# spotify/basic-pitch

Measured on NVIDIA H100. Metric: audio_seconds_per_second, higher is better.
Workload: dtype f32

## Files before the change

### basic_pitch_b200/_lib.py

```python
from __future__ import annotations

import ctypes as C
import os
import pathlib
from typing import Optional

LIB_PATH = pathlib.Path(__file__).resolve().parent / "libbp_b200.so"

BP_OK = 0
BP_E_INVALID = -1
BP_E_CUDA = -2
BP_E_CAPACITY = -3
BP_E_NOMEM = -4

EXPORTS = [
    "bp_version", "bp_last_error", "bp_default_decode_params", "bp_num_windows", "bp_num_frames",
    "bp_model_create", "bp_model_destroy", "bp_model_device", "bp_model_param_block", "bp_model_refresh",
    "bp_model_launch_count", "bp_forward_device", "bp_forward_host", "bp_run_inference_device",
    "bp_run_inference_host", "bp_decode_device", "bp_decode_host", "bp_transcribe_host", "bp_transcribe_device",
    "bp_infer_onsets_host", "bp_pitch_bends_host", "bp_debug_activation", "bp_model_chunk_windows", "bp_model_set_path", "bp_model_profile", "bp_model_profile_read", "bp_debug_tc_plan", "bp_debug_tc_gather", "bp_debug_tc_gather_packed", "bp_debug_tc_b2", "bp_debug_tc_clocks", "bp_transcribe_files_host", "bp_host_alloc", "bp_host_free", "bp_last_required", "bp_resampled_length", "bp_load_pcm_device", "bp_load_pcm_host", "bp_debug_resample_filter", "bp_write_note_files", "bp_sonify_notes_host", "bp_load_pcm_files_device", "bp_transcribe_pcm_files_host", "bp_debug_pcm_layout", "bp_debug_frontend", "bp_model_set_debug_frontend", "bp_debug_chain_layout", "bp_debug_split_layout", "bp_decode_grid_device", "bp_decode_grid_host", "bp_decode_grid_chunk_params", "bp_default_score_params", "bp_frame_times", "bp_score_grid_device", "bp_score_grid_host", "bp_score_notes_host", "bp_multipitch_map", "bp_score_frames_grid_device", "bp_score_frames_grid_host", "bp_score_multipitch_host", "bp_score_salience_grid_device", "bp_score_salience_grid_host", "bp_score_salience_chunk_params", "bp_match_grid_device", "bp_match_grid_host", "bp_match_notes_host", "bp_score_onset_offset_grid_device", "bp_score_onset_offset_grid_host", "bp_score_onset_offset_notes_host",
]


class DecodeParams(C.Structure):
    _fields_ = [
        ("onset_thresh", C.c_double),
        ("frame_thresh", C.c_double),
        ("min_note_len", C.c_int32),
        ("energy_tol", C.c_int32),
        ("infer_onsets", C.c_int32),
        ("melodia_trick", C.c_int32),
        ("include_pitch_bends", C.c_int32),
        ("min_pitch_idx", C.c_int32),
        ("max_pitch_idx", C.c_int32),
        ("reserved", C.c_int32),
# ... 141 lines not shown
                                                  C.POINTER(MultipitchSet), C.c_double, vp, vp, vp, vp]
    lib.bp_score_salience_grid_host.argtypes = [vp, vp, i32, vp, i32, C.POINTER(SalienceParams), i32,
                                                C.POINTER(MultipitchSet), C.c_double, vp, vp, vp]
    lib.bp_score_salience_chunk_params.argtypes = [i64, i64]
    lib.bp_score_salience_chunk_params.restype = i64
    lib.bp_transcribe_host.argtypes = [vp, vp, vp, i32, C.POINTER(DecodeParams), vp, vp, vp, vp, C.POINTER(Notes)]
    lib.bp_transcribe_device.argtypes = [vp, vp, vp, i32, C.POINTER(DecodeParams), vp, C.POINTER(Notes), vp]
    lib.bp_infer_onsets_host.argtypes = [vp, vp, vp, i64, vp]
    lib.bp_pitch_bends_host.argtypes = [vp, vp, i64, i32, vp, vp, vp, vp, vp, i64]
    lib.bp_debug_activation.argtypes = [vp, C.c_int, vp, i64]
    lib.bp_debug_frontend.argtypes = [vp, C.c_int, vp, i64]
    lib.bp_model_set_debug_frontend.argtypes = [vp, C.c_int]
    lib.bp_debug_chain_layout.argtypes = [vp, vp, vp]
    lib.bp_debug_split_layout.argtypes = [vp, vp]
    lib.bp_debug_tc_plan.argtypes = [C.c_int, vp, vp, vp, vp, vp, vp, vp]
    lib.bp_debug_tc_gather.argtypes = [C.c_int, vp, vp, vp, vp, vp]
    lib.bp_debug_tc_gather_packed.argtypes = [C.c_int, vp, vp, vp, vp]
    lib.bp_debug_tc_b2.argtypes = [C.c_int, vp, vp, vp]
    lib.bp_debug_tc_clocks.argtypes = [vp, C.c_int, vp, C.c_int]
    lib.bp_transcribe_files_host.argtypes = [vp, vp, vp, i32, C.POINTER(DecodeParams), vp, vp, vp, vp, C.POINTER(Notes)]
    lib.bp_host_alloc.argtypes = [sz]
    lib.bp_host_alloc.restype = vp
    lib.bp_host_free.argtypes = [vp]
    lib.bp_host_free.restype = None
    lib.bp_last_required.argtypes = [vp, vp]
    lib.bp_last_required.restype = None
    lib.bp_resampled_length.argtypes = [i64, i32]
    lib.bp_resampled_length.restype = i64
    lib.bp_load_pcm_device.argtypes = [vp, vp, i32, i64, i32, i32, vp, vp]
    lib.bp_load_pcm_host.argtypes = [vp, vp, i32, i64, i32, i32, vp]
# ... 23 lines not shown
```

### basic_pitch_b200/csrc/api.cu

```cuda
#include <cuda_runtime.h>

#include <algorithm>
#include <atomic>
#include <chrono>
#include <climits>
#include <cmath>
#include <cstdio>
#include <cstring>
#include <memory>
#include <thread>
#include <string>
#include <vector>

#include "bp_b200.h"
#include "kernels.cuh"

using namespace bp;

namespace {

thread_local std::string g_err;

int fail(int code, const std::string& msg) {
  g_err = msg;
// ... 2810 lines not shown
  byte_off[0] = sample_off[0] = 0;
  for (int i = 0; i < n_files; ++i) {
    byte_off[i + 1] = byte_off[i] + align16(bytes[i]);
    sample_off[i + 1] = sample_off[i] + desc[i].n_out;
  }
  return BP_OK;
}

int64_t bp_debug_resample_filter(int32_t up, int32_t down, double* taps, int64_t capacity) {
  if (up < 1 || down < 1) return fail(BP_E_INVALID, "bp_debug_resample_filter: bad argument"), -1;
  const std::vector<double> h = ingest_filter(up, down);
  if (taps && capacity >= (int64_t)h.size()) std::memcpy(taps, h.data(), h.size() * sizeof(double));
  return (int64_t)h.size();
}

int bp_debug_tc_plan(int which, const float* w, int32_t* sizes, uint16_t* tiles, int32_t* tile_seq, uint32_t* slot_words,
                     int32_t* group_step_off, int32_t* group_ft) {
  if (!w || !sizes || which < 0 || which > 2) return fail(BP_E_INVALID, "bp_debug_tc_plan: bad argument");
  TcConvPlan pl;
  pl.build(tc_spec(which), w);
  sizes[0] = pl.n_tiles;
  sizes[1] = (int32_t)pl.tile_seq.size();
  sizes[2] = pl.n_uses;
  sizes[3] = pl.n_groups;
  if (tiles) std::memcpy(tiles, pl.tiles.data(), pl.tiles.size() * 2);
  if (tile_seq) std::memcpy(tile_seq, pl.tile_seq.data(), pl.tile_seq.size() * 4);
  if (slot_words) {
    std::memcpy(slot_words, pl.slot_words[0].data(), pl.slot_words[0].size() * 4);
    std::memcpy(slot_words + pl.slot_words[0].size(), pl.slot_words[1].data(), pl.slot_words[1].size() * 4);
  }
// ... 192 lines not shown
```

### basic_pitch_b200/csrc/cqt_tc.cu

```cuda
#include <cuda_bf16.h>

#include <cstdio>
#include <cstdlib>
#include <vector>

#include "kernels.cuh"
#include "tc_ptx.cuh"

namespace bp {

namespace cq {
constexpr int kMTile = 128;
constexpr int kKc = 64;
constexpr int kN = 80;
constexpr int kAPlane = (kKc / 8) * kMTile * 16;
constexpr int kWPlane = (kKc / 8) * kN * 16;
constexpr int kStageBytes = 3 * kAPlane + 3 * kWPlane;
constexpr int kStages = 2;
constexpr int kRowsPerWarp = 8;
constexpr int kProducers = 32 * kMTile / kRowsPerWarp;
constexpr int kEpiWarps = 8;
constexpr int kThreads = kProducers + 32 * kEpiWarps;
constexpr int kTilePitch = 37;
constexpr int kStgPitch = 68;
constexpr int kSegOctave = 3;
constexpr int kSegPlane = (kMTile * kStgPitch * 4 / (3 * 2)) & ~7;
static_assert(kSegPlane >= 126 * 32 + 2 * kTaps + 32, "segment of the hop-32 octave");
constexpr int kEpiBytes = kEpiWarps * 16 * kTilePitch * 4;
constexpr int kSmemBytes = kStages * kStageBytes + 256 + kEpiBytes + kMTile * kStgPitch * 4 + kMTile * 24;
static_assert(kThreads <= 1024 && kRowsPerWarp % 2 == 0 && (kKc * kRowsPerWarp / 32) % 8 == 0, "producer geometry");
static_assert(kSmemBytes <= 232448, "shared memory per CTA");
}

static inline uint16_t f2bf_rn(float x) {
  uint32_t u;
  memcpy(&u, &x, 4);
  u += 0x7fffu + ((u >> 16) & 1u);
  return (uint16_t)(u >> 16);
}
static inline float bf2f_(uint16_t h) {
  uint32_t u = (uint32_t)h << 16;
  float f;
  memcpy(&f, &u, 4);
  return f;
}
// ... 5 lines not shown
      const float w = (n & 1) ? cqt_imag[(n >> 1) * kTaps + k] : cqt_real[(n >> 1) * kTaps + k];
      const uint16_t h = f2bf_rn(w);
      const float r1 = w - bf2f_(h);
      const uint16_t m = f2bf_rn(r1);
      const uint16_t l = f2bf_rn(r1 - bf2f_(m));
      const int c = k / cq::kKc, kk = k % cq::kKc;
      const size_t plane = (size_t)8 * cq::kN * 8;
      const size_t base = (size_t)c * 3 * plane;
      const size_t off = ((size_t)(kk >> 3) * cq::kN + n) * 8 + (kk & 7);
      out[base + off] = h;
      out[base + plane + off] = m;
      out[base + 2 * plane + off] = l;
    }
}

struct RowP {
  const float* src;
  int i0, lo, hi, live;
};

struct CqtTcArgs {
  const float* audio;
  const WinDesc* desc;
  const float* chain;
  const uint16_t* wtc;
  const float* scale;
  float* logmag;
  unsigned int* minmax;
  int n_windows, n_mtiles;
};
__global__ void __launch_bounds__(cq::kThreads, 1) cqt_tc_kernel(const CqtTcArgs a) {
  using namespace cq;
  extern __shared__ __align__(128) unsigned char smem[];
  uint64_t* bars = reinterpret_cast<uint64_t*>(smem + kStages * kStageBytes);
  uint64_t* full = bars;
  uint64_t* empty = bars + kStages;

  const int warp = __shfl_sync(0xffffffffu, (int)(threadIdx.x >> 5), 0);
  const int lane = threadIdx.x & 31;

  if (threadIdx.x == 0) {
    for (int s = 0; s < kStages; ++s) {
      mbar_init(full + s, kProducers / 32);
      mbar_init(empty + s, kEpiWarps);
    }
    asm volatile("fence.mbarrier_init.release.cluster;" ::: "memory");
  }
  __syncthreads();

  const int n_items = a.n_mtiles * kOctaves;
  const int total_frames = a.n_windows * kFrames;

  if (warp >= kEpiWarps) {
    constexpr int RW = kRowsPerWarp, NI = RW / 2;
    constexpr int KQ = 32 / RW;
    constexpr int TPL = kKc / KQ;
    const int ptid = threadIdx.x - 32 * kEpiWarps;
    const int pw = ptid >> 5;
    const int r = RW * pw + (lane % RW);
    const int kq = lane / RW;
    float* stg = reinterpret_cast<float*>(smem + kStages * kStageBytes + 256 + kEpiBytes);
    RowP* rowp = reinterpret_cast<RowP*>(smem + kStages * kStageBytes + 256 + kEpiBytes +
                                         kMTile * kStgPitch * 4) + RW * pw;
    uint32_t stage = 0, ph = 0;
        for (int it = blockIdx.x; it < n_items; it += gridDim.x) {
      const int mt = it / kOctaves, o = it % kOctaves;
      const int hop = 256 >> o;
      const int len = octave_len_rt(o);
      asm volatile("bar.sync 1, %0;" ::"n"(kProducers) : "memory");
      if (o >= kSegOctave) {
        __nv_bfloat16* seg = reinterpret_cast<__nv_bfloat16*>(stg);
        const int m0 = mt * kMTile;
        const int b0 = m0 / kFrames, t0 = m0 - b0 * kFrames;
        const int n0 = min(kMTile, kFrames - t0);
        const int s0 = t0 * hop - 128, a0 = s0 & ~7, d0 = s0 - a0;
        const int L0 = ((n0 - 1) * hop + kTaps + d0 + 7) & ~7;
        const int L1 = n0 < kMTile ? (((kMTile - n0 - 1) * hop + kTaps + 7) & ~7) : 0;
        {
          constexpr int NS = (126 * 32 + 2 * kTaps + 32 + kProducers - 1) / kProducers;
          float xs[NS];
#pragma unroll
          for (int q = 0; q < NS; ++q) {
            const int idx = ptid + q * kProducers;
            const int part = idx >= L0;
            const int b = b0 + part;
            int i = part ? idx - L0 - 128 : a0 + idx;
            if (i < 0) i = -i;
            if (i >= len) i = 2 * (len - 1) - i;
            xs[q] = (idx < L0 + L1 && b < a.n_windows && i >= 0 && i < len)
                        ? __ldg(a.chain + (size_t)b * kChainStride + chain_off_rt(o) + i)
                        : 0.f;
          }
#pragma unroll
          for (int q = 0; q < NS; ++q) {
            const int idx = ptid + q * kProducers;
            if (idx < L0 + L1) {
              const float x = xs[q];
              const __nv_bfloat16 h = __float2bfloat16_rn(x);
              const float r1 = x - __bfloat162float(h);
              const __nv_bfloat16 md = __float2bfloat16_rn(r1);
              seg[idx] = h;
              seg[kSegPlane + idx] = md;
              seg[2 * kSegPlane + idx] = __float2bfloat16_rn(r1 - __bfloat162float(md));
            }
          }
        }
        asm volatile("bar.sync 1, %0;" ::"n"(kProducers) : "memory");
        for (int c = 0; c < kTaps / kKc; ++c) {
          mbar_wait(empty + stage, ph ^ 1);
          unsigned char* sa = smem + stage * kStageBytes;
          if (ptid == 0) {
            mbar_expect_tx_only(full + stage, 3 * kWPlane);
            bulk_g2s(sa + 3 * kAPlane, a.wtc + (size_t)c * (3 * kWPlane / 2), 3 * kWPlane, full + stage);
          }
#pragma unroll
          for (int q = 0; q < 3 * 8 * kMTile / kProducers; ++q) {
            const int id = ptid + q * kProducers;
            const int row = id & (kMTile - 1), kc = (id >> 7) & 7, pl = id >> 10;
            const int e = (row < n0 ? d0 + row * hop : L0 + (row - n0) * hop) + c * kKc + kc * 8;
            const __nv_bfloat16* src = seg + pl * kSegPlane + e;
            uint4 v;
            if ((e & 7) == 0) {
              v = *reinterpret_cast<const uint4*>(src);
            } else if ((e & 1) == 0) {
              const uint32_t* w = reinterpret_cast<const uint32_t*>(src);
              v = make_uint4(w[0], w[1], w[2], w[3]);
            } else {
              const uint32_t* w = reinterpret_cast<const uint32_t*>(src - 1);
              v = make_uint4(__funnelshift_r(w[0], w[1], 16), __funnelshift_r(w[1], w[2], 16),
                             __funnelshift_r(w[2], w[3], 16), __funnelshift_r(w[3], w[4], 16));
            }
            *reinterpret_cast<uint4*>(sa + pl * kAPlane + (kc * kMTile + row) * 16) = v;
          }
          asm volatile("fence.proxy.async.shared::cta;" ::: "memory");
          __syncwarp();
          if (lane == 0) mbar_arrive(full + stage);
          if (++stage == kStages) {
            stage = 0;
            ph ^= 1;
          }
        }
        continue;
      }
      __syncwarp();
      if (lane < RW) {
        const int m = mt * kMTile + RW * pw + lane;
        RowP p;
        p.live = m < total_frames;
        const int b = p.live ? m / kFrames : 0;
        const int t = m - b * kFrames;
        p.lo = 0;
        p.hi = len;
        if (o == 0) {
          if (a.desc) {
            const WinDesc d = a.desc[b];
            p.src = a.audio + d.base;
            p.lo = d.lo;
            p.hi = d.hi;
          } else {
            p.src = a.audio + (long long)b * kWinSamples;
          }
        } else {
          p.src = a.chain + (size_t)b * kChainStride + chain_off_rt(o);
        }
        p.i0 = t * hop - 128;
        rowp[lane] = p;
      }
      __syncwarp();
      for (int c = 0; c < kTaps / kKc; ++c) {
        float xs[4 * NI];
        unsigned vmask = 0;
#pragma unroll
        for (int i = 0; i < NI; ++i) {
          const RowP p = rowp[2 * i + (lane >> 4)];
          const int ibv = p.i0 + c * kKc;
          const bool okv = p.live && ibv >= p.lo && ibv + kKc <= p.hi && ibv >= 0 && ibv + kKc <= len &&
                           ((reinterpret_cast<uintptr_t>(p.src + ibv) & 15) == 0);
          if (__all_sync(0xffffffffu, okv)) {
            vmask |= 1u << i;
            const float4 v = __ldg(reinterpret_cast<const float4*>(p.src + ibv) + (lane & 15));
            xs[4 * i] = v.x, xs[4 * i + 1] = v.y, xs[4 * i + 2] = v.z, xs[4 * i + 3] = v.w;
          } else {
#pragma unroll
            for (int q = 0; q < 4; ++q) {
              const RowP pq = rowp[2 * i + (q >> 1)];
              int idx = pq.i0 + c * kKc + (q & 1) * 32 + lane;
              float xv = 0.f;
              if (pq.live) {
                if (idx < 0) idx = -idx;
                if (idx >= len) idx = 2 * (len - 1) - idx;
                if (idx >= pq.lo && idx < pq.hi) xv = __ldg(pq.src + idx);
              }
              xs[4 * i + q] = xv;
            }
          }
        }
        __syncwarp();
#pragma unroll
        for (int i = 0; i < NI; ++i) {
          if ((vmask >> i) & 1u) {
            *reinterpret_cast<float4*>(stg + (RW * pw + 2 * i + (lane >> 4)) * kStgPitch + 4 * (lane & 15)) =
                make_float4(xs[4 * i], xs[4 * i + 1], xs[4 * i + 2], xs[4 * i + 3]);
          } else {
#pragma unroll
            for (int q = 0; q < 4; ++q)
              stg[(RW * pw + 2 * i + (q >> 1)) * kStgPitch + (q & 1) * 32 + lane] = xs[4 * i + q];
          }
        }
        __syncwarp();
        float xb[TPL];
        {
          const float4* sp = reinterpret_cast<const float4*>(stg + r * kStgPitch + TPL * kq);
#pragma unroll
          for (int i = 0; i < TPL / 4; ++i) {
            const float4 v = sp[i];
            xb[4 * i] = v.x, xb[4 * i + 1] = v.y, xb[4 * i + 2] = v.z, xb[4 * i + 3] = v.w;
          }
        }
        mbar_wait(empty + stage, ph ^ 1);
        unsigned char* sa = smem + stage * kStageBytes;
        if (ptid == 0) {
          mbar_expect_tx_only(full + stage, 3 * kWPlane);
          bulk_g2s(sa + 3 * kAPlane, a.wtc + (size_t)c * (3 * kWPlane / 2), 3 * kWPlane, full + stage);
        }
#pragma unroll
        for (int q = 0; q < TPL / 8; ++q) {
          const int kc = kq * (TPL / 8) + q;
          const float* x = xb + 8 * q;
          __align__(16) __nv_bfloat162 h[4], md[4], l[4];
#pragma unroll
          for (int j = 0; j < 4; ++j) {
            h[j] = __floats2bfloat162_rn(x[2 * j], x[2 * j + 1]);
            const float2 hf = __bfloat1622float2(h[j]);
            const float r0 = x[2 * j] - hf.x, r1 = x[2 * j + 1] - hf.y;
            md[j] = __floats2bfloat162_rn(r0, r1);
            const float2 mf = __bfloat1622float2(md[j]);
            l[j] = __floats2bfloat162_rn(r0 - mf.x, r1 - mf.y);
          }
          const int o16 = (kc * kMTile + r) * 16;
          *reinterpret_cast<uint4*>(sa + o16) = *reinterpret_cast<const uint4*>(h);
          *reinterpret_cast<uint4*>(sa + kAPlane + o16) = *reinterpret_cast<const uint4*>(md);
          *reinterpret_cast<uint4*>(sa + 2 * kAPlane + o16) = *reinterpret_cast<const uint4*>(l);
        }
        asm volatile("fence.proxy.async.shared::cta;" ::: "memory");
        __syncwarp();
        if (lane == 0) mbar_arrive(full + stage);
        if (++stage == kStages) {
          stage = 0;
          ph ^= 1;
        }
      }
    }
  } else {
    const int h = warp >> 2, w = warp & 3, g = lane >> 2, q = lane & 3;
    const int r0 = 64 * h + 16 * w + g;
    uint32_t stage = 0, ph = 0;
    float* tile = reinterpret_cast<float*>(smem + kStages * kStageBytes + 256) + warp * (16 * kTilePitch);
    for (int it = blockIdx.x; it < n_items; it += gridDim.x) {
      const int mt = it / kOctaves, o = it % kOctaves;
      float d[kN / 2];
#pragma unroll
      for (int i = 0; i < kN / 2; ++i) d[i] = 0.f;
      for (int c = 0; c < kTaps / kKc; ++c) {
        mbar_wait(full + stage, ph);
        const uint32_t sa = smem_u32(smem + stage * kStageBytes);
        wgmma_fence();
#pragma unroll
        for (int ks = 0; ks < kKc / 16; ++ks) {
          const uint32_t ao = sa + (uint32_t)(ks * 2 * (kMTile * 16) + h * 64 * 16);
          const uint32_t bo = sa + 3 * kAPlane + (uint32_t)(ks * 2 * (kN * 16));
          uint64_t A[3], B[3];
#pragma unroll
          for (int p = 0; p < 3; ++p) {
            A[p] = make_desc(ao + p * kAPlane, kMTile * 16, 128);
            B[p] = make_desc(bo + p * kWPlane, kN * 16, 128);
          }
          wgmma_ss_n80(d, A[0], B[0], (c | ks) ? 1u : 0u);
          wgmma_ss_n80(d, A[0], B[1], 1u);
          wgmma_ss_n80(d, A[1], B[0], 1u);
          wgmma_ss_n80(d, A[0], B[2], 1u);
          wgmma_ss_n80(d, A[2], B[0], 1u);
          wgmma_ss_n80(d, A[1], B[1], 1u);
        }
        wgmma_commit();
        wgmma_wait<0>();
        reg_fence(d);
        __syncwarp();
        if (lane == 0) mbar_arrive(empty + stage);
        if (++stage == kStages) {
          stage = 0;
          ph ^= 1;
        }
      }
      const int gb0 = (8 - o) * kBinsPerOctave - 15;
      float vmin[2] = {INFINITY, INFINITY}, vmax[2] = {-INFINITY, -INFINITY};
      int bw[2];
#pragma unroll
      for (int rr = 0; rr < 2; ++rr) {
        const int m = mt * kMTile + r0 + 8 * rr;
        const bool live = m < total_frames;
        bw[rr] = live ? m / kFrames : -1;
#pragma unroll
        for (int i = 0; i < 9; ++i) {
          const int bin = 4 * i + q, gg = gb0 + bin;
          float L = 0.f;
          if (gg >= 0) {
            const float s = __ldg(a.scale + gg);
            const float re = d[4 * i + 2 * rr] * s, im = d[4 * i + 2 * rr + 1] * s;
            L = __log2f(fmaf(re, re, im * im) + 1e-10f) * 3.0102999566398120f;
            if (live) {
              vmin[rr] = fminf(vmin[rr], L);
              vmax[rr] = fmaxf(vmax[rr], L);
            }
          }
          tile[(g + 8 * rr) * kTilePitch + bin] = L;
        }
      }
      __syncwarp();
      {
        const int m0 = mt * kMTile + 64 * h + 16 * w;
        for (int e = lane; e < 16 * kBinsPerOctave; e += 32) {
          const int rr = e / kBinsPerOctave, jj = e - rr * kBinsPerOctave;
          if (m0 + rr < total_frames && gb0 + jj >= 0) a.logmag[(size_t)(m0 + rr) * kCqtBins + gb0 + jj] = tile[rr * kTilePitch + jj];
        }
      }
      __syncwarp();
      const int b0 = __shfl_sync(0xffffffffu, bw[0], 0);
      const bool uniform = __all_sync(0xffffffffu, bw[0] == b0 && bw[1] == b0);
      if (uniform) {
        if (b0 >= 0) {
          float mn = fminf(vmin[0], vmin[1]), mx = fmaxf(vmax[0], vmax[1]);
#pragma unroll
          for (int off = 16; off; off >>= 1) {
            mn = fminf(mn, __shfl_xor_sync(0xffffffffu, mn, off));
            mx = fmaxf(mx, __shfl_xor_sync(0xffffffffu, mx, off));
          }
          if (lane == 0 && mn <= mx) {
            atomicMin(a.minmax + 2 * b0, float_to_ordered(mn));
            atomicMax(a.minmax + 2 * b0 + 1, float_to_ordered(mx));
          }
        }
      } else {
#pragma unroll
        for (int rr = 0; rr < 2; ++rr)
          if (bw[rr] >= 0 && vmin[rr] <= vmax[rr]) {
            atomicMin(a.minmax + 2 * bw[rr], float_to_ordered(vmin[rr]));
            atomicMax(a.minmax + 2 * bw[rr] + 1, float_to_ordered(vmax[rr]));
          }
      }
    }
  }
}

__global__ void minmax_init_kernel2(unsigned int* mm, int n) {
  int i = blockIdx.x * blockDim.x + threadIdx.x;
  if (i < n) {
    mm[2 * i] = 0xffffffffu;
    mm[2 * i + 1] = 0u;
  }
}

void cqt_tc_setup() { cudaFuncSetAttribute(cqt_tc_kernel, cudaFuncAttributeMaxDynamicSharedMemorySize, cq::kSmemBytes); }

void launch_cqt_tc(const float* audio, const WinDesc* desc, const float* chain, const uint16_t* wtc, const float* scale,
                   float* logmag, unsigned int* minmax, int n_windows, int n_sms, cudaStream_t st) {
  minmax_init_kernel2<<<(n_windows + 255) / 256, 256, 0, st>>>(minmax, n_windows);
  CqtTcArgs a;
  a.audio = audio;
  a.desc = desc;
  a.chain = chain;
  a.wtc = wtc;
  a.scale = scale;
  a.logmag = logmag;
  a.minmax = minmax;
  a.n_windows = n_windows;
  a.n_mtiles = (n_windows * kFrames + cq::kMTile - 1) / cq::kMTile;
  const int n_items = a.n_mtiles * kOctaves;
  const int grid = n_items < n_sms ? n_items : n_sms;
  cqt_tc_kernel<<<grid, cq::kThreads, cq::kSmemBytes, st>>>(a);
}

}
```

### basic_pitch_b200/csrc/kernels.cuh

```cuda
#pragma once
#include <cuda_bf16.h>

#include <cstring>
#include <vector>

#include "common.cuh"

namespace bp {

void hcqt_setup();
constexpr int kLp2 = kTaps + 14;
struct Lowpass2 {
  float2 t[kLp2];
};
Lowpass2 lowpass_pairs(const float* h_lp );
void launch_decimate(const Lowpass2& lp, const float* audio, const WinDesc* desc, float* chain, int stage, int n_windows,
                     cudaStream_t st);
void launch_cqt(const float* audio, const WinDesc* desc, const float* chain, const float* wt, const float* scale,
                float* logmag, unsigned int* minmax, int n_windows, cudaStream_t st);
void launch_lognorm(float* y, const unsigned int* minmax, const float* bn , int n_windows,
                    cudaStream_t st);

struct CnnWeights {
  const float *contour1_wT, *contour1_b;
// ... 112 lines not shown
  float* unwrapped = nullptr;
  long long frame_stride = 0;
  long long raw_rows = 0;
  const UnwrapDesc* ud = nullptr;
  const float* note_raw = nullptr;
  __nv_bfloat16* chl = nullptr;
  int chl_rows = 0, chl_chunks = 0, chl_rpw = 0, chl_lead = 0;
  float* edge = nullptr;
  float* act = nullptr;
};
void launch_conv_tc(const __nv_bfloat16* data, const TcConvDev& dev, const TcOut& out, int n_windows, int rows_stride,
                    int n_sms, cudaStream_t st, bool fuse_next = false);
void launch_contour2_tc(const float* c1_nhwc, const CnnWeights& w, float* contour, __nv_bfloat16* chl, int rows_total,
                        int n_windows, cudaStream_t st);

void build_cqt_tc_weights(const float* cqt_real, const float* cqt_imag, std::vector<uint16_t>& out);
void cqt_tc_setup();
void launch_cqt_tc(const float* audio, const WinDesc* desc, const float* chain, const uint16_t* wtc, const float* scale,
                   float* logmag, unsigned int* minmax, int n_windows, int n_sms, cudaStream_t st);

void launch_rows_to_pm(const float* rows, long long n_frames, int width, float* pm, long long stride, long long dst_frame0,
                       cudaStream_t st, const UnwrapDesc* ud = nullptr, int n_windows = 0);
void launch_rows_to_cm(const float* rows, long long n_frames, float* cm, long long stride, long long dst_frame0,
                       cudaStream_t st, const UnwrapDesc* ud = nullptr, int n_windows = 0);
void launch_pm_to_rows(const float* pm, long long stride, long long src_frame0, long long n_frames, int width, float* rows,
                       cudaStream_t st);
void launch_cm_to_rows(const float* cm, long long stride, long long src_frame0, long long n_frames, float* rows,
                       cudaStream_t st);

long long ingest_output_length(long long n_frames, int sample_rate);
std::vector<double> ingest_filter(int up, int down);
int launch_ingest(int device, const void* d_pcm, int format, long long n_frames, int channels, int sample_rate, float* d_out,
// ... 156 lines not shown
```

### include/bp_b200.h

```cpp
#ifndef BP_B200_H
#define BP_B200_H

#include <stddef.h>
#include <stdint.h>

#ifdef __cplusplus
extern "C" {
#endif

#define BP_OK 0
#define BP_E_INVALID (-1)
#define BP_E_CUDA (-2)
#define BP_E_CAPACITY (-3)
#define BP_E_NOMEM (-4)

#define BP_SAMPLE_RATE 22050
#define BP_WINDOW_SAMPLES 43844
#define BP_WINDOW_FRAMES 172
#define BP_N_PITCHES 88
#define BP_N_CONTOUR_BINS 264
#define BP_OVERLAP_FRAMES 30
#define BP_HOP_SAMPLES 36164
#define BP_HOP_FRAMES 142
#define BP_LEAD_ZEROS 3840
// ... 196 lines not shown
                                 int64_t* h_frame_off, int64_t* h_sample_off, bp_notes_t* notes);
int bp_debug_pcm_layout(const bp_pcm_file_t* files, int32_t n_files, int64_t* byte_off, int64_t* sample_off);

int bp_write_note_files(int32_t n_files, const char* const* midi_paths, const char* const* csv_paths,
                        const int32_t* note_off, const double* start_s, const double* end_s, const int32_t* pitch_midi,
                        const float* amplitude, const int32_t* bend_off, const int32_t* bends,
                        int32_t multiple_pitch_bends, double midi_tempo, int32_t n_threads);

int bp_sonify_notes_host(bp_model_t* m, int32_t n_files, const int32_t* note_off, const double* start_s,
                         const double* end_s, const int32_t* pitch_midi, const float* amplitude, const int32_t* bend_off,
                         const int32_t* bends, int32_t multiple_pitch_bends, int32_t sample_rate, int64_t* h_sample_off,
                         double* h_audio, int64_t capacity);

int64_t bp_debug_resample_filter(int32_t up, int32_t down, double* taps, int64_t capacity);

int bp_debug_tc_plan(int which, const float* w, int32_t* sizes, uint16_t* tiles, int32_t* tile_seq, uint32_t* slot_words,
                     int32_t* group_step_off, int32_t* group_ft);

int bp_debug_tc_gather(int which, const float* w, int32_t* sizes, uint16_t* b1, int32_t* starts, int32_t* ranges);
int bp_debug_tc_gather_packed(int which, const float* w, int32_t* sizes, uint16_t* b1, int32_t* kmap);

int bp_debug_tc_b2(int which, const float* w2, int32_t* sizes, uint16_t* tiles);

int bp_model_profile(bp_model_t* m, int which);
int bp_model_profile_read(bp_model_t* m, double* total_ms, int64_t* n_intervals, int64_t* n_windows);

int bp_debug_tc_clocks(bp_model_t* m, int which, uint64_t* cycles, int reset);

#ifdef __cplusplus
}
// ... 3 lines not shown
```

Measured before the change: 147,800.

## Restructure CQT tensor-core kernel around per-window items with phase-strided A layout

The CQT wgmma kernel now processes one window-octave item per iteration and builds a phase-interleaved A operand where overlapping frame rows share sample chunks. The old approach staged a bf16 segment in shared memory and re-gathered it per k-chunk. The full weight matrix is now loaded once per CTA into shared memory instead of being streamed per stage. Producers load float4 samples directly from global memory, split them into three bf16 planes, and feed 12 consumer warps. Per-window min/max atomics become uniform per warp. This trades more shared memory for weights against less redundant gathering and weight traffic. It also adds a debug export for the layout.

```diff
diff --git a/basic_pitch_b200/_lib.py b/basic_pitch_b200/_lib.py
--- a/basic_pitch_b200/_lib.py
+++ b/basic_pitch_b200/_lib.py
@@ -18,7 +18,7 @@
     "bp_model_create", "bp_model_destroy", "bp_model_device", "bp_model_param_block", "bp_model_refresh",
     "bp_model_launch_count", "bp_forward_device", "bp_forward_host", "bp_run_inference_device",
     "bp_run_inference_host", "bp_decode_device", "bp_decode_host", "bp_transcribe_host", "bp_transcribe_device",
-    "bp_infer_onsets_host", "bp_pitch_bends_host", "bp_debug_activation", "bp_model_chunk_windows", "bp_model_set_path", "bp_model_profile", "bp_model_profile_read", "bp_debug_tc_plan", "bp_debug_tc_gather", "bp_debug_tc_gather_packed", "bp_debug_tc_b2", "bp_debug_tc_clocks", "bp_transcribe_files_host", "bp_host_alloc", "bp_host_free", "bp_last_required", "bp_resampled_length", "bp_load_pcm_device", "bp_load_pcm_host", "bp_debug_resample_filter", "bp_write_note_files", "bp_sonify_notes_host", "bp_load_pcm_files_device", "bp_transcribe_pcm_files_host", "bp_debug_pcm_layout", "bp_debug_frontend", "bp_model_set_debug_frontend", "bp_debug_chain_layout", "bp_debug_split_layout", "bp_decode_grid_device", "bp_decode_grid_host", "bp_decode_grid_chunk_params", "bp_default_score_params", "bp_frame_times", "bp_score_grid_device", "bp_score_grid_host", "bp_score_notes_host", "bp_multipitch_map", "bp_score_frames_grid_device", "bp_score_frames_grid_host", "bp_score_multipitch_host", "bp_score_salience_grid_device", "bp_score_salience_grid_host", "bp_score_salience_chunk_params", "bp_match_grid_device", "bp_match_grid_host", "bp_match_notes_host", "bp_score_onset_offset_grid_device", "bp_score_onset_offset_grid_host", "bp_score_onset_offset_notes_host",
+    "bp_infer_onsets_host", "bp_pitch_bends_host", "bp_debug_activation", "bp_model_chunk_windows", "bp_model_set_path", "bp_model_profile", "bp_model_profile_read", "bp_debug_tc_plan", "bp_debug_cqt_layout", "bp_debug_tc_gather", "bp_debug_tc_gather_packed", "bp_debug_tc_b2", "bp_debug_tc_clocks", "bp_transcribe_files_host", "bp_host_alloc", "bp_host_free", "bp_last_required", "bp_resampled_length", "bp_load_pcm_device", "bp_load_pcm_host", "bp_debug_resample_filter", "bp_write_note_files", "bp_sonify_notes_host", "bp_load_pcm_files_device", "bp_transcribe_pcm_files_host", "bp_debug_pcm_layout", "bp_debug_frontend", "bp_model_set_debug_frontend", "bp_debug_chain_layout", "bp_debug_split_layout", "bp_decode_grid_device", "bp_decode_grid_host", "bp_decode_grid_chunk_params", "bp_default_score_params", "bp_frame_times", "bp_score_grid_device", "bp_score_grid_host", "bp_score_notes_host", "bp_multipitch_map", "bp_score_frames_grid_device", "bp_score_frames_grid_host", "bp_score_multipitch_host", "bp_score_salience_grid_device", "bp_score_salience_grid_host", "bp_score_salience_chunk_params", "bp_match_grid_device", "bp_match_grid_host", "bp_match_notes_host", "bp_score_onset_offset_grid_device", "bp_score_onset_offset_grid_host", "bp_score_onset_offset_notes_host",
 ]
 
 
@@ -190,6 +190,7 @@
     lib.bp_debug_chain_layout.argtypes = [vp, vp, vp]
     lib.bp_debug_split_layout.argtypes = [vp, vp]
     lib.bp_debug_tc_plan.argtypes = [C.c_int, vp, vp, vp, vp, vp, vp, vp]
+    lib.bp_debug_cqt_layout.argtypes = [i32, i32, i32, vp, vp, vp]
     lib.bp_debug_tc_gather.argtypes = [C.c_int, vp, vp, vp, vp, vp]
     lib.bp_debug_tc_gather_packed.argtypes = [C.c_int, vp, vp, vp, vp]
     lib.bp_debug_tc_b2.argtypes = [C.c_int, vp, vp, vp]
diff --git a/basic_pitch_b200/csrc/api.cu b/basic_pitch_b200/csrc/api.cu
--- a/basic_pitch_b200/csrc/api.cu
+++ b/basic_pitch_b200/csrc/api.cu
@@ -2848,6 +2848,32 @@
   return (int64_t)h.size();
 }
 
+int bp_debug_cqt_layout(int32_t octave, int32_t lo, int32_t hi, int32_t* geom, int32_t* desc, int32_t* samples) {
+  if (!geom || octave < 0 || octave >= kOctaves) return fail(BP_E_INVALID, "bp_debug_cqt_layout: bad argument");
+  const int o = octave, nb = cqt_blocks(o), nks = cqt_block_ksteps(o), len = octave_len(o);
+  const int32_t g[10] = {nb, nks, cqt_phases(o), cqt_rows(o), cqt_rows_used(o), cqt_plane_bytes(o), cqt_block_bytes(o),
+                         cqt_stage_bytes(), cqt_tc_smem_bytes(), len};
+  std::memcpy(geom, g, sizeof(g));
+  if (desc)
+    for (int mt = 0; mt < 3; ++mt)
+      for (int ks = 0; ks < nks; ++ks) {
+        int32_t* d = desc + 3 * (mt * nks + ks);
+        d[0] = cqt_a_start(o, mt, ks);
+        d[1] = cqt_lbo(o);
+        d[2] = 128;
+      }
+  if (samples) {
+    const int n = cqt_plane_bytes(o) / 2;
+    for (int blk = 0; blk < nb; ++blk)
+      for (int e = 0; e < n; ++e) {
+        const int p = e / (8 * cqt_rows(o)), r = e / 8 % cqt_rows(o);
+        samples[(size_t)blk * n + e] =
+            r < cqt_rows_used(o) ? cqt_source(cqt_sample(o, blk, p, r) + e % 8, len, lo, hi) : -2;
+      }
+  }
+  return BP_OK;
+}
+
 int bp_debug_tc_plan(int which, const float* w, int32_t* sizes, uint16_t* tiles, int32_t* tile_seq, uint32_t* slot_words,
                      int32_t* group_step_off, int32_t* group_ft) {
   if (!w || !sizes || which < 0 || which > 2) return fail(BP_E_INVALID, "bp_debug_tc_plan: bad argument");
diff --git a/basic_pitch_b200/csrc/cqt_tc.cu b/basic_pitch_b200/csrc/cqt_tc.cu
--- a/basic_pitch_b200/csrc/cqt_tc.cu
+++ b/basic_pitch_b200/csrc/cqt_tc.cu
@@ -10,25 +10,30 @@
 namespace bp {
 
 namespace cq {
-constexpr int kMTile = 128;
 constexpr int kKc = 64;
 constexpr int kN = 80;
-constexpr int kAPlane = (kKc / 8) * kMTile * 16;
 constexpr int kWPlane = (kKc / 8) * kN * 16;
-constexpr int kStageBytes = 3 * kAPlane + 3 * kWPlane;
+constexpr int kWBytes = (kTaps / kKc) * 3 * kWPlane;
+constexpr int kStageBytes = cqt_stage_bytes();
 constexpr int kStages = 2;
-constexpr int kRowsPerWarp = 8;
-constexpr int kProducers = 32 * kMTile / kRowsPerWarp;
-constexpr int kEpiWarps = 8;
-constexpr int kThreads = kProducers + 32 * kEpiWarps;
+constexpr int kConsumerWarps = 12;
+constexpr int kProducerThreads = 128;
+constexpr int kThreads = 32 * kConsumerWarps + kProducerThreads;
+constexpr int kUnits = 4 * 199;
+constexpr int kUnitsPerThread = (kUnits + kProducerThreads - 1) / kProducerThreads;
 constexpr int kTilePitch = 37;
-constexpr int kStgPitch = 68;
-constexpr int kSegOctave = 3;
-constexpr int kSegPlane = (kMTile * kStgPitch * 4 / (3 * 2)) & ~7;
-static_assert(kSegPlane >= 126 * 32 + 2 * kTaps + 32, "segment of the hop-32 octave");
-constexpr int kEpiBytes = kEpiWarps * 16 * kTilePitch * 4;
-constexpr int kSmemBytes = kStages * kStageBytes + 256 + kEpiBytes + kMTile * kStgPitch * 4 + kMTile * 24;
-static_assert(kThreads <= 1024 && kRowsPerWarp % 2 == 0 && (kKc * kRowsPerWarp / 32) % 8 == 0, "producer geometry");
+constexpr int kEpiBytes = kConsumerWarps * 16 * kTilePitch * 4;
+constexpr int kStageOff = kWBytes;
+constexpr int kEpiOff = kStageOff + kStages * kStageBytes;
+constexpr int kBarOff = kEpiOff + kEpiBytes;
+constexpr int kSmemBytes = kBarOff + 8 * (2 * kStages + 1);
+__host__ __device__ constexpr bool units_fit() {
+  for (int o = 0; o < kOctaves; ++o)
+    if (cqt_phases(o) * cqt_rows_used(o) > kUnits) return false;
+  return true;
+}
+static_assert(units_fit(), "producer units of a block");
+static_assert(kStageBytes % 128 == 0 && kEpiOff % 16 == 0 && kBarOff % 8 == 0, "shared-memory alignment");
 static_assert(kSmemBytes <= 232448, "shared memory per CTA");
 }
 
@@ -64,10 +69,29 @@
     }
 }
 
-struct RowP {
-  const float* src;
-  int i0, lo, hi, live;
-};
+template <int NKS>
+__device__ __forceinline__ void mma_block(float (&d)[cq::kN / 2], uint32_t sa, uint32_t wsm, int o, int mt, int ks0,
+                                          uint32_t lbo, uint32_t plane) {
+  using namespace cq;
+#pragma unroll
+  for (int kl = 0; kl < NKS; ++kl) {
+    const int ks = ks0 + kl;
+    const uint32_t ao = sa + (uint32_t)cqt_a_start(o, mt, kl);
+    const uint32_t bo = wsm + (uint32_t)((ks >> 2) * 3 * kWPlane + (ks & 3) * 2 * (kN * 16));
+    uint64_t A[3], B[3];
+#pragma unroll
+    for (int p = 0; p < 3; ++p) {
+      A[p] = make_desc(ao + p * plane, lbo, 128);
+      B[p] = make_desc(bo + p * kWPlane, kN * 16, 128);
+    }
+    wgmma_ss_n80(d, A[0], B[0], ks ? 1u : 0u);
+    wgmma_ss_n80(d, A[0], B[1], 1u);
+    wgmma_ss_n80(d, A[1], B[0], 1u);
+    wgmma_ss_n80(d, A[0], B[2], 1u);
+    wgmma_ss_n80(d, A[2], B[0], 1u);
+    wgmma_ss_n80(d, A[1], B[1], 1u);
+  }
+}
 
 struct CqtTcArgs {
   const float* audio;
@@ -77,279 +101,151 @@
   const float* scale;
   float* logmag;
   unsigned int* minmax;
-  int n_windows, n_mtiles;
+  int n_windows;
 };
 __global__ void __launch_bounds__(cq::kThreads, 1) cqt_tc_kernel(const CqtTcArgs a) {
   using namespace cq;
   extern __shared__ __align__(128) unsigned char smem[];
-  uint64_t* bars = reinterpret_cast<uint64_t*>(smem + kStages * kStageBytes);
-  uint64_t* full = bars;
-  uint64_t* empty = bars + kStages;
+  uint64_t* full = reinterpret_cast<uint64_t*>(smem + kBarOff);
+  uint64_t* empty = full + kStages;
+  uint64_t* wbar = empty + kStages;
 
   const int warp = __shfl_sync(0xffffffffu, (int)(threadIdx.x >> 5), 0);
   const int lane = threadIdx.x & 31;
 
   if (threadIdx.x == 0) {
     for (int s = 0; s < kStages; ++s) {
-      mbar_init(full + s, kProducers / 32);
-      mbar_init(empty + s, kEpiWarps);
-    }
+      mbar_init(full + s, kProducerThreads / 32);
+      mbar_init(empty + s, kConsumerWarps);
+    }
+    mbar_init(wbar, 1);
     asm volatile("fence.mbarrier_init.release.cluster;" ::: "memory");
   }
   __syncthreads();
 
-  const int n_items = a.n_mtiles * kOctaves;
-  const int total_frames = a.n_windows * kFrames;
-
-  if (warp >= kEpiWarps) {
-    constexpr int RW = kRowsPerWarp, NI = RW / 2;
-    constexpr int KQ = 32 / RW;
-    constexpr int TPL = kKc / KQ;
-    const int ptid = threadIdx.x - 32 * kEpiWarps;
-    const int pw = ptid >> 5;
-    const int r = RW * pw + (lane % RW);
-    const int kq = lane / RW;
-    float* stg = reinterpret_cast<float*>(smem + kStages * kStageBytes + 256 + kEpiBytes);
-    RowP* rowp = reinterpret_cast<RowP*>(smem + kStages * kStageBytes + 256 + kEpiBytes +
-                                         kMTile * kStgPitch * 4) + RW * pw;
-    uint32_t stage = 0, ph = 0;
-        for (int it = blockIdx.x; it < n_items; it += gridDim.x) {
-      const int mt = it / kOctaves, o = it % kOctaves;
-      const int hop = 256 >> o;
+  const int n_items = a.n_windows * kOctaves;
+
+  if (warp >= kConsumerWarps) {
+    const int ptid = threadIdx.x - 32 * kConsumerWarps;
+    if (ptid == 0) {
+      mbar_expect_tx(wbar, kWBytes);
+      for (int c = 0; c < kTaps / kKc; ++c)
+        bulk_g2s(smem + c * 3 * kWPlane, a.wtc + (size_t)c * (3 * kWPlane / 2), 3 * kWPlane, wbar);
+    }
+    uint32_t n = 0;
+    for (int it = blockIdx.x; it < n_items; it += gridDim.x) {
+      const int b = it / kOctaves, o = it - b * kOctaves;
       const int len = octave_len_rt(o);
-      asm volatile("bar.sync 1, %0;" ::"n"(kProducers) : "memory");
-      if (o >= kSegOctave) {
-        __nv_bfloat16* seg = reinterpret_cast<__nv_bfloat16*>(stg);
-        const int m0 = mt * kMTile;
-        const int b0 = m0 / kFrames, t0 = m0 - b0 * kFrames;
-        const int n0 = min(kMTile, kFrames - t0);
-        const int s0 = t0 * hop - 128, a0 = s0 & ~7, d0 = s0 - a0;
-        const int L0 = ((n0 - 1) * hop + kTaps + d0 + 7) & ~7;
-        const int L1 = n0 < kMTile ? (((kMTile - n0 - 1) * hop + kTaps + 7) & ~7) : 0;
-        {
-          constexpr int NS = (126 * 32 + 2 * kTaps + 32 + kProducers - 1) / kProducers;
-          float xs[NS];
-#pragma unroll
-          for (int q = 0; q < NS; ++q) {
-            const int idx = ptid + q * kProducers;
-            const int part = idx >= L0;
-            const int b = b0 + part;
-            int i = part ? idx - L0 - 128 : a0 + idx;
-            if (i < 0) i = -i;
-            if (i >= len) i = 2 * (len - 1) - i;
-            xs[q] = (idx < L0 + L1 && b < a.n_windows && i >= 0 && i < len)
-                        ? __ldg(a.chain + (size_t)b * kChainStride + chain_off_rt(o) + i)
-                        : 0.f;
-          }
-#pragma unroll
-          for (int q = 0; q < NS; ++q) {
-            const int idx = ptid + q * kProducers;
-            if (idx < L0 + L1) {
-              const float x = xs[q];
-              const __nv_bfloat16 h = __float2bfloat16_rn(x);
-              const float r1 = x - __bfloat162float(h);
-              const __nv_bfloat16 md = __float2bfloat16_rn(r1);
-              seg[idx] = h;
-              seg[kSegPlane + idx] = md;
-              seg[2 * kSegPlane + idx] = __float2bfloat16_rn(r1 - __bfloat162float(md));
+      const int P = cqt_phases(o), lgP = cqt_lg_phases(o), rows = cqt_rows(o);
+      const int units = P * cqt_rows_used(o), plane = cqt_plane_bytes(o);
+      const float* src;
+      int lo = 0, hi = len;
+      if (o == 0) {
+        if (a.desc) {
+          const WinDesc d = a.desc[b];
+          src = a.audio + d.base;
+          lo = d.lo;
+          hi = d.hi;
+        } else {
+          src = a.audio + (long long)b * kWinSamples;
+        }
+      } else {
+        src = a.chain + (size_t)b * kChainStride + chain_off_rt(o);
+      }
+      for (int blk = 0; blk < cqt_blocks(o); ++blk, ++n) {
+        const uint32_t stage = n % kStages, ph = (n / kStages) & 1;
+        float x[kUnitsPerThread][8];
+#pragma unroll
+        for (int i = 0; i < kUnitsPerThread; ++i) {
+          const int u = ptid + i * kProducerThreads;
+          const int s = cqt_sample(o, blk, u & (P - 1), u >> lgP);
+          if (u < units) {
+            if (s >= 0 && s >= lo && s + 8 <= len && s + 8 <= hi && (reinterpret_cast<uintptr_t>(src + s) & 15) == 0) {
+              const float4 v0 = __ldg(reinterpret_cast<const float4*>(src + s));
+              const float4 v1 = __ldg(reinterpret_cast<const float4*>(src + s) + 1);
+              x[i][0] = v0.x, x[i][1] = v0.y, x[i][2] = v0.z, x[i][3] = v0.w;
+              x[i][4] = v1.x, x[i][5] = v1.y, x[i][6] = v1.z, x[i][7] = v1.w;
+              if (o <= 2 && blk + 1 < cqt_blocks(o) && s + 40 <= len && s + 40 <= hi)
+                asm volatile("prefetch.global.L2 [%0];" ::"l"(src + s + 32));
+            } else {
+#pragma unroll
+              for (int e = 0; e < 8; ++e) {
+                const int j = cqt_source(s + e, len, lo, hi);
+                x[i][e] = j >= 0 ? __ldg(src + j) : 0.f;
+              }
             }
           }
         }
-        asm volatile("bar.sync 1, %0;" ::"n"(kProducers) : "memory");
-        for (int c = 0; c < kTaps / kKc; ++c) {
-          mbar_wait(empty + stage, ph ^ 1);
-          unsigned char* sa = smem + stage * kStageBytes;
-          if (ptid == 0) {
-            mbar_expect_tx_only(full + stage, 3 * kWPlane);
-            bulk_g2s(sa + 3 * kAPlane, a.wtc + (size_t)c * (3 * kWPlane / 2), 3 * kWPlane, full + stage);
+        mbar_wait(empty + stage, ph ^ 1);
+        unsigned char* sa = smem + kStageOff + stage * kStageBytes;
+#pragma unroll
+        for (int i = 0; i < kUnitsPerThread; ++i) {
+          const int u = ptid + i * kProducerThreads;
+          if (u < units) {
+            __align__(16) __nv_bfloat162 h[4], md[4], l[4];
+#pragma unroll
+            for (int j = 0; j < 4; ++j) {
+              h[j] = __floats2bfloat162_rn(x[i][2 * j], x[i][2 * j + 1]);
+              const float2 hf = __bfloat1622float2(h[j]);
+              const float r0 = x[i][2 * j] - hf.x, r1 = x[i][2 * j + 1] - hf.y;
+              md[j] = __floats2bfloat162_rn(r0, r1);
+              const float2 mf = __bfloat1622float2(md[j]);
+              l[j] = __floats2bfloat162_rn(r0 - mf.x, r1 - mf.y);
+            }
+            const int o16 = ((u & (P - 1)) * rows + (u >> lgP)) * 16;
+            *reinterpret_cast<uint4*>(sa + o16) = *reinterpret_cast<const uint4*>(h);
+            *reinterpret_cast<uint4*>(sa + plane + o16) = *reinterpret_cast<const uint4*>(md);
+            *reinterpret_cast<uint4*>(sa + 2 * plane + o16) = *reinterpret_cast<const uint4*>(l);
           }
-#pragma unroll
-          for (int q = 0; q < 3 * 8 * kMTile / kProducers; ++q) {
-            const int id = ptid + q * kProducers;
-            const int row = id & (kMTile - 1), kc = (id >> 7) & 7, pl = id >> 10;
-            const int e = (row < n0 ? d0 + row * hop : L0 + (row - n0) * hop) + c * kKc + kc * 8;
-            const __nv_bfloat16* src = seg + pl * kSegPlane + e;
-            uint4 v;
-            if ((e & 7) == 0) {
-              v = *reinterpret_cast<const uint4*>(src);
-            } else if ((e & 1) == 0) {
-              const uint32_t* w = reinterpret_cast<const uint32_t*>(src);
-              v = make_uint4(w[0], w[1], w[2], w[3]);
-            } else {
-              const uint32_t* w = reinterpret_cast<const uint32_t*>(src - 1);
-              v = make_uint4(__funnelshift_r(w[0], w[1], 16), __funnelshift_r(w[1], w[2], 16),
-                             __funnelshift_r(w[2], w[3], 16), __funnelshift_r(w[3], w[4], 16));
-            }
-            *reinterpret_cast<uint4*>(sa + pl * kAPlane + (kc * kMTile + row) * 16) = v;
-          }
-          asm volatile("fence.proxy.async.shared::cta;" ::: "memory");
-          __syncwarp();
-          if (lane == 0) mbar_arrive(full + stage);
-          if (++stage == kStages) {
-            stage = 0;
-            ph ^= 1;
-          }
-        }
-        continue;
-      }
-      __syncwarp();
-      if (lane < RW) {
-        const int m = mt * kMTile + RW * pw + lane;
-        RowP p;
-        p.live = m < total_frames;
-        const int b = p.live ? m / kFrames : 0;
-        const int t = m - b * kFrames;
-        p.lo = 0;
-        p.hi = len;
-        if (o == 0) {
-          if (a.desc) {
-            const WinDesc d = a.desc[b];
-            p.src = a.audio + d.base;
-            p.lo = d.lo;
-            p.hi = d.hi;
-          } else {
-            p.src = a.audio + (long long)b * kWinSamples;
-          }
-        } else {
-          p.src = a.chain + (size_t)b * kChainStride + chain_off_rt(o);
-        }
-        p.i0 = t * hop - 128;
-        rowp[lane] = p;
-      }
-      __syncwarp();
-      for (int c = 0; c < kTaps / kKc; ++c) {
-        float xs[4 * NI];
-        unsigned vmask = 0;
-#pragma unroll
-        for (int i = 0; i < NI; ++i) {
-          const RowP p = rowp[2 * i + (lane >> 4)];
-          const int ibv = p.i0 + c * kKc;
-          const bool okv = p.live && ibv >= p.lo && ibv + kKc <= p.hi && ibv >= 0 && ibv + kKc <= len &&
-                           ((reinterpret_cast<uintptr_t>(p.src + ibv) & 15) == 0);
-          if (__all_sync(0xffffffffu, okv)) {
-            vmask |= 1u << i;
-            const float4 v = __ldg(reinterpret_cast<const float4*>(p.src + ibv) + (lane & 15));
-            xs[4 * i] = v.x, xs[4 * i + 1] = v.y, xs[4 * i + 2] = v.z, xs[4 * i + 3] = v.w;
-          } else {
-#pragma unroll
-            for (int q = 0; q < 4; ++q) {
-              const RowP pq = rowp[2 * i + (q >> 1)];
-              int idx = pq.i0 + c * kKc + (q & 1) * 32 + lane;
-              float xv = 0.f;
-              if (pq.live) {
-                if (idx < 0) idx = -idx;
-                if (idx >= len) idx = 2 * (len - 1) - idx;
-                if (idx >= pq.lo && idx < pq.hi) xv = __ldg(pq.src + idx);
-              }
-              xs[4 * i + q] = xv;
-            }
-          }
-        }
-        __syncwarp();
-#pragma unroll
-        for (int i = 0; i < NI; ++i) {
-          if ((vmask >> i) & 1u) {
-            *reinterpret_cast<float4*>(stg + (RW * pw + 2 * i + (lane >> 4)) * kStgPitch + 4 * (lane & 15)) =
-                make_float4(xs[4 * i], xs[4 * i + 1], xs[4 * i + 2], xs[4 * i + 3]);
-          } else {
-#pragma unroll
-            for (int q = 0; q < 4; ++q)
-              stg[(RW * pw + 2 * i + (q >> 1)) * kStgPitch + (q & 1) * 32 + lane] = xs[4 * i + q];
-          }
-        }
-        __syncwarp();
-        float xb[TPL];
-        {
-          const float4* sp = reinterpret_cast<const float4*>(stg + r * kStgPitch + TPL * kq);
-#pragma unroll
-          for (int i = 0; i < TPL / 4; ++i) {
-            const float4 v = sp[i];
-            xb[4 * i] = v.x, xb[4 * i + 1] = v.y, xb[4 * i + 2] = v.z, xb[4 * i + 3] = v.w;
-          }
-        }
-        mbar_wait(empty + stage, ph ^ 1);
-        unsigned char* sa = smem + stage * kStageBytes;
-        if (ptid == 0) {
-          mbar_expect_tx_only(full + stage, 3 * kWPlane);
-          bulk_g2s(sa + 3 * kAPlane, a.wtc + (size_t)c * (3 * kWPlane / 2), 3 * kWPlane, full + stage);
-        }
-#pragma unroll
-        for (int q = 0; q < TPL / 8; ++q) {
-          const int kc = kq * (TPL / 8) + q;
-          const float* x = xb + 8 * q;
-          __align__(16) __nv_bfloat162 h[4], md[4], l[4];
-#pragma unroll
-          for (int j = 0; j < 4; ++j) {
-            h[j] = __floats2bfloat162_rn(x[2 * j], x[2 * j + 1]);
-            const float2 hf = __bfloat1622float2(h[j]);
-            const float r0 = x[2 * j] - hf.x, r1 = x[2 * j + 1] - hf.y;
-            md[j] = __floats2bfloat162_rn(r0, r1);
-            const float2 mf = __bfloat1622float2(md[j]);
-            l[j] = __floats2bfloat162_rn(r0 - mf.x, r1 - mf.y);
-          }
-          const int o16 = (kc * kMTile + r) * 16;
-          *reinterpret_cast<uint4*>(sa + o16) = *reinterpret_cast<const uint4*>(h);
-          *reinterpret_cast<uint4*>(sa + kAPlane + o16) = *reinterpret_cast<const uint4*>(md);
-          *reinterpret_cast<uint4*>(sa + 2 * kAPlane + o16) = *reinterpret_cast<const uint4*>(l);
         }
         asm volatile("fence.proxy.async.shared::cta;" ::: "memory");
         __syncwarp();
         if (lane == 0) mbar_arrive(full + stage);
+      }
+    }
+  } else {
+    const int mt = warp >> 2, w = warp & 3, g = lane >> 2, q = lane & 3;
+    const int t0 = 64 * mt + 16 * w;
+    const uint32_t wsm = smem_u32(smem);
+    float* tile = reinterpret_cast<float*>(smem + kEpiOff) + warp * (16 * kTilePitch);
+    mbar_wait(wbar, 0);
+    uint32_t stage = 0, ph = 0;
+    for (int it = blockIdx.x; it < n_items; it += gridDim.x) {
+      const int b = it / kOctaves, o = it - b * kOctaves;
+      const uint32_t lbo = cqt_lbo(o), plane = cqt_plane_bytes(o);
+      float d[kN / 2];
+#pragma unroll
+      for (int i = 0; i < kN / 2; ++i) d[i] = 0.f;
+      uint32_t prev = 0;
+      for (int blk = 0; blk < cqt_blocks(o); ++blk) {
+        mbar_wait(full + stage, ph);
+        const uint32_t sa = wsm + kStageOff + stage * kStageBytes;
+        wgmma_fence();
+        if (o <= 2)
+          mma_block<2>(d, sa, wsm, o, mt, blk * 2, lbo, plane);
+        else
+          mma_block<16>(d, sa, wsm, o, mt, 0, lbo, plane);
+        wgmma_commit();
+        if (blk > 0) {
+          wgmma_wait<1>();
+          __syncwarp();
+          if (lane == 0) mbar_arrive(empty + prev);
+        }
+        prev = stage;
         if (++stage == kStages) {
           stage = 0;
           ph ^= 1;
         }
       }
-    }
-  } else {
-    const int h = warp >> 2, w = warp & 3, g = lane >> 2, q = lane & 3;
-    const int r0 = 64 * h + 16 * w + g;
-    uint32_t stage = 0, ph = 0;
-    float* tile = reinterpret_cast<float*>(smem + kStages * kStageBytes + 256) + warp * (16 * kTilePitch);
-    for (int it = blockIdx.x; it < n_items; it += gridDim.x) {
-      const int mt = it / kOctaves, o = it % kOctaves;
-      float d[kN / 2];
-#pragma unroll
-      for (int i = 0; i < kN / 2; ++i) d[i] = 0.f;
-      for (int c = 0; c < kTaps / kKc; ++c) {
-        mbar_wait(full + stage, ph);
-        const uint32_t sa = smem_u32(smem + stage * kStageBytes);
-        wgmma_fence();
-#pragma unroll
-        for (int ks = 0; ks < kKc / 16; ++ks) {
-          const uint32_t ao = sa + (uint32_t)(ks * 2 * (kMTile * 16) + h * 64 * 16);
-          const uint32_t bo = sa + 3 * kAPlane + (uint32_t)(ks * 2 * (kN * 16));
-          uint64_t A[3], B[3];
-#pragma unroll
-          for (int p = 0; p < 3; ++p) {
-            A[p] = make_desc(ao + p * kAPlane, kMTile * 16, 128);
-            B[p] = make_desc(bo + p * kWPlane, kN * 16, 128);
-          }
-          wgmma_ss_n80(d, A[0], B[0], (c | ks) ? 1u : 0u);
-          wgmma_ss_n80(d, A[0], B[1], 1u);
-          wgmma_ss_n80(d, A[1], B[0], 1u);
-          wgmma_ss_n80(d, A[0], B[2], 1u);
-          wgmma_ss_n80(d, A[2], B[0], 1u);
-          wgmma_ss_n80(d, A[1], B[1], 1u);
-        }
-        wgmma_commit();
-        wgmma_wait<0>();
-        reg_fence(d);
-        __syncwarp();
-        if (lane == 0) mbar_arrive(empty + stage);
-        if (++stage == kStages) {
-          stage = 0;
-          ph ^= 1;
-        }
-      }
+      wgmma_wait<0>();
+      reg_fence(d);
+      __syncwarp();
+      if (lane == 0) mbar_arrive(empty + prev);
       const int gb0 = (8 - o) * kBinsPerOctave - 15;
-      float vmin[2] = {INFINITY, INFINITY}, vmax[2] = {-INFINITY, -INFINITY};
-      int bw[2];
+      float vmin = INFINITY, vmax = -INFINITY;
 #pragma unroll
       for (int rr = 0; rr < 2; ++rr) {
-        const int m = mt * kMTile + r0 + 8 * rr;
-        const bool live = m < total_frames;
-        bw[rr] = live ? m / kFrames : -1;
+        const bool live = t0 + g + 8 * rr < kFrames;
 #pragma unroll
         for (int i = 0; i < 9; ++i) {
           const int bin = 4 * i + q, gg = gb0 + bin;
@@ -359,44 +255,30 @@
             const float re = d[4 * i + 2 * rr] * s, im = d[4 * i + 2 * rr + 1] * s;
             L = __log2f(fmaf(re, re, im * im) + 1e-10f) * 3.0102999566398120f;
             if (live) {
-              vmin[rr] = fminf(vmin[rr], L);
-              vmax[rr] = fmaxf(vmax[rr], L);
+              vmin = fminf(vmin, L);
+              vmax = fmaxf(vmax, L);
             }
           }
           tile[(g + 8 * rr) * kTilePitch + bin] = L;
         }
       }
       __syncwarp();
-      {
-        const int m0 = mt * kMTile + 64 * h + 16 * w;
+      if (t0 < kFrames) {
+        float* dst = a.logmag + ((size_t)b * kFrames + t0) * kCqtBins + gb0;
         for (int e = lane; e < 16 * kBinsPerOctave; e += 32) {
           const int rr = e / kBinsPerOctave, jj = e - rr * kBinsPerOctave;
-          if (m0 + rr < total_frames && gb0 + jj >= 0) a.logmag[(size_t)(m0 + rr) * kCqtBins + gb0 + jj] = tile[rr * kTilePitch + jj];
+          if (t0 + rr < kFrames && gb0 + jj >= 0) dst[(size_t)rr * kCqtBins + jj] = tile[rr * kTilePitch + jj];
         }
       }
       __syncwarp();
-      const int b0 = __shfl_sync(0xffffffffu, bw[0], 0);
-      const bool uniform = __all_sync(0xffffffffu, bw[0] == b0 && bw[1] == b0);
-      if (uniform) {
-        if (b0 >= 0) {
-          float mn = fminf(vmin[0], vmin[1]), mx = fmaxf(vmax[0], vmax[1]);
-#pragma unroll
-          for (int off = 16; off; off >>= 1) {
-            mn = fminf(mn, __shfl_xor_sync(0xffffffffu, mn, off));
-            mx = fmaxf(mx, __shfl_xor_sync(0xffffffffu, mx, off));
-          }
-          if (lane == 0 && mn <= mx) {
-            atomicMin(a.minmax + 2 * b0, float_to_ordered(mn));
-            atomicMax(a.minmax + 2 * b0 + 1, float_to_ordered(mx));
-          }
-        }
-      } else {
-#pragma unroll
-        for (int rr = 0; rr < 2; ++rr)
-          if (bw[rr] >= 0 && vmin[rr] <= vmax[rr]) {
-            atomicMin(a.minmax + 2 * bw[rr], float_to_ordered(vmin[rr]));
-            atomicMax(a.minmax + 2 * bw[rr] + 1, float_to_ordered(vmax[rr]));
-          }
+#pragma unroll
+      for (int off = 16; off; off >>= 1) {
+        vmin = fminf(vmin, __shfl_xor_sync(0xffffffffu, vmin, off));
+        vmax = fmaxf(vmax, __shfl_xor_sync(0xffffffffu, vmax, off));
+      }
+      if (lane == 0 && vmin <= vmax) {
+        atomicMin(a.minmax + 2 * b, float_to_ordered(vmin));
+        atomicMax(a.minmax + 2 * b + 1, float_to_ordered(vmax));
       }
     }
   }
@@ -411,6 +293,8 @@
 }
 
 void cqt_tc_setup() { cudaFuncSetAttribute(cqt_tc_kernel, cudaFuncAttributeMaxDynamicSharedMemorySize, cq::kSmemBytes); }
+
+int cqt_tc_smem_bytes() { return cq::kSmemBytes; }
 
 void launch_cqt_tc(const float* audio, const WinDesc* desc, const float* chain, const uint16_t* wtc, const float* scale,
                    float* logmag, unsigned int* minmax, int n_windows, int n_sms, cudaStream_t st) {
@@ -424,8 +308,7 @@
   a.logmag = logmag;
   a.minmax = minmax;
   a.n_windows = n_windows;
-  a.n_mtiles = (n_windows * kFrames + cq::kMTile - 1) / cq::kMTile;
-  const int n_items = a.n_mtiles * kOctaves;
+  const int n_items = n_windows * kOctaves;
   const int grid = n_items < n_sms ? n_items : n_sms;
   cqt_tc_kernel<<<grid, cq::kThreads, cq::kSmemBytes, st>>>(a);
 }
diff --git a/basic_pitch_b200/csrc/kernels.cuh b/basic_pitch_b200/csrc/kernels.cuh
--- a/basic_pitch_b200/csrc/kernels.cuh
+++ b/basic_pitch_b200/csrc/kernels.cuh
@@ -150,8 +150,41 @@
 void launch_contour2_tc(const float* c1_nhwc, const CnnWeights& w, float* contour, __nv_bfloat16* chl, int rows_total,
                         int n_windows, cudaStream_t st);
 
+constexpr int kCqtItemRows = 192;
+__host__ __device__ constexpr int cqt_blocks(int o) { return o <= 2 ? 8 : 1; }
+__host__ __device__ constexpr int cqt_block_ksteps(int o) { return 16 / cqt_blocks(o); }
+__host__ __device__ constexpr int cqt_phases(int o) { return o <= 3 ? 4 : o == 4 ? 2 : 1; }
+__host__ __device__ constexpr int cqt_lg_phases(int o) { return o <= 3 ? 2 : o == 4 ? 1 : 0; }
+__host__ __device__ constexpr int cqt_row_step(int o) { return o <= 5 ? 16 : 16 * (8 >> (8 - o)); }
+__host__ __device__ constexpr int cqt_rows_used(int o) {
+  return kCqtItemRows + (2 * cqt_block_ksteps(o) - 1) / cqt_phases(o) * (cqt_row_step(o) / 16);
+}
+__host__ __device__ constexpr int cqt_rows(int o) {
+  return cqt_phases(o) == 1 ? cqt_rows_used(o) : cqt_rows_used(o) + ((8 / cqt_phases(o) - cqt_rows_used(o)) % 8 + 8) % 8;
+}
+__host__ __device__ constexpr int cqt_plane_bytes(int o) { return cqt_phases(o) * cqt_rows(o) * 16; }
+__host__ __device__ constexpr int cqt_block_bytes(int o) { return 3 * cqt_plane_bytes(o); }
+__host__ __device__ constexpr int cqt_stage_bytes() {
+  int m = 0;
+  for (int o = 0; o < kOctaves; ++o) m = cqt_block_bytes(o) > m ? cqt_block_bytes(o) : m;
+  return m;
+}
+__host__ __device__ constexpr int cqt_sample(int o, int blk, int p, int r) {
+  return r * (256 >> o) + 8 * p + 32 * blk - 128;
+}
+__host__ __device__ constexpr int cqt_a_start(int o, int mt, int ks) {
+  return ((2 * ks) & (cqt_phases(o) - 1)) * cqt_rows(o) * 16 + ((2 * ks) >> cqt_lg_phases(o)) * cqt_row_step(o) +
+         64 * mt * 16;
+}
+__host__ __device__ constexpr int cqt_lbo(int o) { return cqt_phases(o) > 1 ? cqt_rows(o) * 16 : cqt_row_step(o); }
+__host__ __device__ constexpr int cqt_source(int i, int len, int lo, int hi) {
+  i = i < 0 ? -i : i;
+  i = i >= len ? 2 * (len - 1) - i : i;
+  return (i >= 0 && i < len && i >= lo && i < hi) ? i : -1;
+}
 void build_cqt_tc_weights(const float* cqt_real, const float* cqt_imag, std::vector<uint16_t>& out);
 void cqt_tc_setup();
+int cqt_tc_smem_bytes();
 void launch_cqt_tc(const float* audio, const WinDesc* desc, const float* chain, const uint16_t* wtc, const float* scale,
                    float* logmag, unsigned int* minmax, int n_windows, int n_sms, cudaStream_t st);
 
diff --git a/include/bp_b200.h b/include/bp_b200.h
--- a/include/bp_b200.h
+++ b/include/bp_b200.h
@@ -234,6 +234,8 @@
 
 int64_t bp_debug_resample_filter(int32_t up, int32_t down, double* taps, int64_t capacity);
 
+int bp_debug_cqt_layout(int32_t octave, int32_t lo, int32_t hi, int32_t* geom, int32_t* desc, int32_t* samples);
+
 int bp_debug_tc_plan(int which, const float* w, int32_t* sizes, uint16_t* tiles, int32_t* tile_seq, uint32_t* slot_words,
                      int32_t* group_step_off, int32_t* group_ft);
 
```

Measured after the change: 149,500 (median of 6 runs). 1.01x the previous value.
